# nadeemlab/DeepLIIF

Hardware: AMD Instinct MI355X
Metric: 512x512 tiles/s train-step (5G+5D) (higher is better)
Workload: dtype bf16; 1 GPU; DeepLIIF train step, 5x Resnet-9block G + 5x NLayerD(n=4), GAN+SmoothL1+Adam (BASELINE configs[2] per GPU); tile=512x512x3, batch_per_gpu=8, global_batch=8, norm=instance, precision_policy=bf16, parallelism=dp1, rccl_ranks=1, backend=nccl, streams=3

## Files before the change

deepliif_amd/csrc/wgrad.hip:

```cpp
#include "common.h"
#include <stdlib.h>

typedef __attribute__((ext_vector_type(4))) short s16x4_t;

struct WgradArgs {
    const void *P;
    const void *Q;
    float *slab;
    int kstride;
    int N, Hp, Wp, CAp, p_pstride;
    int Hq, Wq, CBp, log2CB, q_pstride;
    int KH, KW, step, pad, pad_w, pad_mode;
    int J;
    int Ptot;
    int splitk, pchunk;
    int tiles_a, tiles_j;
    int dn, dh, dw;
    int p_act, q_act;
    int xcd_group;
    int p_split, q_split;
    int tr_asm;
};

constexpr int WGRAD_MULTI_MAX = DL_WGRAD_MULTI_MAX;
// ... 601 lines not shown
    DL_CHECK_LAUNCH("dl_conv_wgrad(8-phase)");
    return 0;
}

template <int BA, int WA, int WJ, bool TRASM>
static int launch_wgrad_glds_v(WgradArgs a, const WgradLayers &lay, int n, hipStream_t stream) {
    constexpr size_t smem = (size_t)2 * 64 * (BA + 256) * sizeof(bf16_t);
    a.tiles_a = a.CAp / BA;
    a.tiles_j = (a.J + 255) / 256;
    a.pchunk = ((a.Ptot + a.splitk - 1) / a.splitk + 63) / 64 * 64;
    const int hw = a.Hp * a.Wp;
    a.dn = 64 / hw; a.dh = (64 % hw) / a.Wp; a.dw = (64 % hw) % a.Wp;
    auto kern = wgrad_glds_kernel<BA, WA, WJ, TRASM>;
    static bool attr_set = false;
    if (!attr_set) {
        hipError_t e = hipFuncSetAttribute(reinterpret_cast<const void *>(kern), hipFuncAttributeMaxDynamicSharedMemorySize, (int)smem);
        if (e != hipSuccess) DL_FAIL("dl_conv_wgrad: hipFuncSetAttribute: %s", hipGetErrorString(e));
        attr_set = true;
    }
    hipLaunchKernelGGL(kern, dim3(a.tiles_a * a.tiles_j, a.splitk, n), dim3(512), smem, stream, a, lay);
    DL_CHECK_LAUNCH("dl_conv_wgrad(glds)");
    return 0;
}

template <int BA, int WA, int WJ>
static int launch_wgrad_glds(const WgradArgs &a, const WgradLayers &lay, int n, hipStream_t stream) {
    return a.tr_asm ? launch_wgrad_glds_v<BA, WA, WJ, true>(a, lay, n, stream) : launch_wgrad_glds_v<BA, WA, WJ, false>(a, lay, n, stream);
}

__device__ __forceinline__ void wgrad_reduce_body(const float *slab, int splitk, int kstride_, int CBp, int J, int CA, int CB, int KK, float *grad,
                                                  int accumulate, int stack_kw, int bid, int nb) {
    const int J4 = J / 4;
    const size_t total = (size_t)CA * J4;
    const size_t kstride = (size_t)kstride_;
    for (size_t i = bid * (size_t)blockDim.x + threadIdx.x; i < total; i += (size_t)nb * blockDim.x) {
        const int ca = (int)(i / J4), j = (int)(i % J4) * 4;
        const float *src = slab + (size_t)ca * J + j;
        f32x4_t s = {0.f, 0.f, 0.f, 0.f};
        int k = 0;
        for (; k + 8 <= splitk; k += 8) {
            f32x4_t v[8];
#pragma unroll
            for (int u = 0; u < 8; ++u) v[u] = __builtin_nontemporal_load(reinterpret_cast<const f32x4_t *>(src + (size_t)(k + u) * kstride));
#pragma unroll
            for (int u = 0; u < 8; ++u) s += v[u];
        }
        for (; k < splitk; ++k) s += __builtin_nontemporal_load(reinterpret_cast<const f32x4_t *>(src + (size_t)k * kstride));
        const int t = j / CBp, b0 = j % CBp;
        if (t >= KK) continue;
#pragma unroll
        for (int e = 0; e < 4; ++e) {
            const int b = b0 + e;
            if (b >= CB) continue;
            float *g = stack_kw ? grad + (((size_t)(ca / stack_kw) * CB + b) * KK + t) * stack_kw + (ca % stack_kw)
                                : grad + ((size_t)ca * CB + b) * KK + t;
            *g = accumulate ? *g + s[e] : s[e];
        }
    }
}

constexpr int RED_BCHUNK = 64, RED_KK_MAX = 64, RED_MAX_BLOCKS = 8192;

__device__ __forceinline__ bool wgrad_reduce_tiled(int KK, int stack_kw) { return stack_kw == 0 && KK <= RED_KK_MAX; }

__device__ __forceinline__ void wgrad_reduce_tiles(const float *slab, int splitk, int kstride_, int CBp, int J, int CA, int CB, int KK, float *grad,
                                                   int accumulate, int bid, int nb, float *lds) {
    const int nbc = (CBp + RED_BCHUNK - 1) / RED_BCHUNK, KP = KK + 1;
    const size_t kstride = (size_t)kstride_;
    for (int item = bid; item < CA * nbc; item += nb) {
        const int ca = item / nbc, b0 = (item - ca * nbc) * RED_BCHUNK;
        const int width = min(RED_BCHUNK, CBp - b0), q = width / 4;
        const int nreal = min(width, CB - b0);
        if (nreal > 0) {
            const float *base = slab + (size_t)ca * J + b0;
            for (int i = threadIdx.x; i < KK * q; i += 256) {
                const int t = i / q, c = (i - t * q) * 4;
                const float *src = base + (size_t)t * CBp + c;
                f32x4_t s = {0.f, 0.f, 0.f, 0.f};
                int k = 0;
                for (; k + 8 <= splitk; k += 8) {
                    f32x4_t v[8];
#pragma unroll
                    for (int u = 0; u < 8; ++u) v[u] = __builtin_nontemporal_load(reinterpret_cast<const f32x4_t *>(src + (size_t)(k + u) * kstride));
#pragma unroll
                    for (int u = 0; u < 8; ++u) s += v[u];
                }
                for (; k < splitk; ++k) s += __builtin_nontemporal_load(reinterpret_cast<const f32x4_t *>(src + (size_t)k * kstride));
#pragma unroll
                for (int e = 0; e < 4; ++e) lds[(c + e) * KP + t] = s[e];
            }
        }
        __syncthreads();
        if (nreal > 0) {
            float *g = grad + ((size_t)ca * CB + b0) * KK;
            for (int o = threadIdx.x; o < nreal * KK; o += 256) {
                const float v = lds[o + o / KK];
                g[o] = accumulate ? g[o] + v : v;
            }
        }
        __syncthreads();
    }
}

__global__ void __launch_bounds__(256) wgrad_reduce_kernel(const float *slab, int splitk, int kstride, int CBp, int J, int CA, int CB,
                                                           int KK, float *grad, int accumulate, int stack_kw) {
    __shared__ float lds[RED_BCHUNK * (RED_KK_MAX + 1)];
    if (wgrad_reduce_tiled(KK, stack_kw)) wgrad_reduce_tiles(slab, splitk, kstride, CBp, J, CA, CB, KK, grad, accumulate, blockIdx.x, gridDim.x, lds);
    else wgrad_reduce_body(slab, splitk, kstride, CBp, J, CA, CB, KK, grad, accumulate, stack_kw, blockIdx.x, gridDim.x);
}

__global__ void __launch_bounds__(256) wgrad_reduce_batch_kernel(const dl_wgrad_reduce_entry *tab, int n) {
    __shared__ float lds[RED_BCHUNK * (RED_KK_MAX + 1)];
    int lo = 0, hi = n - 1;
    const int b = blockIdx.x;
    while (lo < hi) {
        const int mid = (lo + hi + 1) >> 1;
        if (tab[mid].block0 <= b) lo = mid; else hi = mid - 1;
    }
    const dl_wgrad_reduce_entry e = tab[lo];
    if (wgrad_reduce_tiled(e.KK, e.stack_kw))
        wgrad_reduce_tiles(e.slab, e.splitk, e.kstride, e.CBp, e.J, e.CA, e.CB, e.KK, e.grad, e.accumulate, b - e.block0, e.nblocks, lds);
    else wgrad_reduce_body(e.slab, e.splitk, e.kstride, e.CBp, e.J, e.CA, e.CB, e.KK, e.grad, e.accumulate, e.stack_kw, b - e.block0, e.nblocks);
}

template <typename T, int PREC, int BA, int WA, int WJ>
static int launch_wgrad(WgradArgs a, hipStream_t stream) {
    constexpr int NPL = (PREC == 3) ? 2 : 1;
    constexpr size_t smem = (size_t)2 * NPL * 32 * ((BA + 16) + (128 + 16)) * sizeof(bf16_t);
    a.tiles_a = (a.CAp + BA - 1) / BA;
    a.tiles_j = (a.J + 127) / 128;
    auto kern = wgrad_kernel<T, PREC, BA, WA, WJ>;
    static bool attr_set = false;
    if (!attr_set) {
        hipError_t e = hipFuncSetAttribute(reinterpret_cast<const void *>(kern), hipFuncAttributeMaxDynamicSharedMemorySize, (int)smem);
        if (e != hipSuccess) DL_FAIL("dl_conv_wgrad: hipFuncSetAttribute: %s", hipGetErrorString(e));
        attr_set = true;
    }
    hipLaunchKernelGGL(kern, dim3(a.tiles_a * a.tiles_j, a.splitk), dim3(256), smem, stream, a);
    DL_CHECK_LAUNCH("dl_conv_wgrad");
    return 0;
}

template <typename T, int PREC>
static int dispatch_wgrad(const WgradArgs &a, hipStream_t stream) {
    if (a.CAp <= 16) return launch_wgrad<T, PREC, 16, 1, 4>(a, stream);
    if (a.CAp <= 32) return launch_wgrad<T, PREC, 32, 1, 4>(a, stream);
    if (a.CAp <= 64) return launch_wgrad<T, PREC, 64, 2, 2>(a, stream);
    return launch_wgrad<T, PREC, 128, 2, 2>(a, stream);
}

#include "wgrad_c4.h"
#include "wgrad_x3.h"
#include "wgrad_w4.h"

static int wgrad_slab_pad() {
    static const int pad = [] { const char *e = DL_DEV_ENV("DL_WGRAD_SLAB_PAD"); const int v = e ? atoi(e) : 0; return v < 0 ? 0 : (v + 3) / 4 * 4; }();
    return pad;
}

extern "C" size_t dl_wgrad_slab_floats(const dl_wgrad_desc *d) {
    if (!d || d->splitk < 1) return 0;
    return (size_t)d->splitk * ((size_t)d->CAp * d->KH * d->KW * d->CBp + wgrad_slab_pad());
}

enum WgradKernel { WK_GENERIC = 0, WK_GLDS256, WK_GLDS128, WK_X3_256, WK_X3_128, WK_8PH, WK_4PH_X3, WK_4PH_X3_NOPRIO, WK_W4 };

static int wgrad_kernel_of(const dl_wgrad_desc *d, int *err) {
    *err = 0;
    const int J = d->KH * d->KW * d->CBp;
    const long Ptot = (long)d->N * d->Hp * d->Wp;
    static const bool no_glds = DL_DEV_ENV("DL_NO_GLDS") != nullptr;
    const bool fast = d->dtype == DL_BF16 && d->prec == DL_PREC_BF16 && d->p_act == DL_ACT_NONE && d->q_act == DL_ACT_NONE &&
                      d->pad_mode == DL_PAD_ZERO && J >= 256 && Ptot >= 64L * d->splitk && !no_glds;
    static const char *w8 = DL_DEV_ENV("DL_WGRAD_8PH");
    const bool no_x3 = dl_switch(DL_SW_NO_X3_GLDS) != nullptr;
    const bool act_ok3 = (d->p_act == DL_ACT_NONE || d->p_act == DL_ACT_RELU || d->p_act == DL_ACT_LRELU) &&
                         (d->q_act == DL_ACT_NONE || d->q_act == DL_ACT_RELU || d->q_act == DL_ACT_LRELU);
    const bool fast3 = d->dtype == DL_F32 && d->prec == DL_PREC_BF16X3 && act_ok3 && d->pad_mode == DL_PAD_ZERO && J >= 256 &&
                       Ptot >= 32L * d->splitk && (d->p_pstride % 4) == 0 && (d->q_pstride % 4) == 0 && !no_x3;
    static const char *w3 = DL_DEV_ENV("DL_WGRAD_X3");
    if ((d->p_split || d->q_split) && !(fast3 && (d->CAp % 128) == 0 && (!d->p_split || d->p_act == DL_ACT_NONE) && (!d->q_split || d->q_act == DL_ACT_NONE))) {
        *err = 1;
        return WK_GENERIC;
    }
    if (w4w_eligible(d)) return WK_W4;
    if (fast3 && (d->CAp % 256) == 0 && w3 && (w3[0] == '2' || w3[0] == '3') && !d->p_split && !d->q_split) return w3[0] == '3' ? WK_4PH_X3_NOPRIO : WK_4PH_X3;
    if (fast3 && (d->CAp % 256) == 0) return WK_X3_256;
    if (fast3 && (d->CAp % 128) == 0) return WK_X3_128;
    if (fast && (d->CAp % 256) == 0 && w8 && w8[0] == '1') return WK_8PH;
    if (fast && (d->CAp % 256) == 0) return WK_GLDS256;
    if (fast && (d->CAp % 128) == 0) return WK_GLDS128;
    return WK_GENERIC;
}

static int wgrad_slabs(const dl_wgrad_desc *d, const WgradLayers &lay, int n, hipStream_t stream, int *J_out) {
    if (!d) DL_FAIL("dl_conv_wgrad: null descriptor");
    if (d->N <= 0 || d->Hp <= 0 || d->Wp <= 0 || d->Hq <= 0 || d->Wq <= 0)
        DL_FAIL("dl_conv_wgrad: empty problem (N=%d, P %dx%d, Q %dx%d): nothing to launch", d->N, d->Hp, d->Wp, d->Hq, d->Wq);
    if (n < 1 || n > WGRAD_MULTI_MAX) DL_FAIL("dl_conv_wgrad: %d layers in one launch (1 .. %d)", n, WGRAD_MULTI_MAX);
    for (int l = 0; l < n; ++l)
        if (!lay.P[l] || !lay.Q[l] || !lay.slab[l]) DL_FAIL("dl_conv_wgrad: null argument");
    const int l2 = ilog2_exact(d->CBp);
    if (l2 < 3) DL_FAIL("dl_conv_wgrad: CBp=%d must be a power of two >= 8", d->CBp);
    if (d->CAp % 8) DL_FAIL("dl_conv_wgrad: CAp=%d must be a multiple of 8", d->CAp);
    if (d->p_pstride % 8 || d->q_pstride % 8) DL_FAIL("dl_conv_wgrad: pixel strides must be multiples of 8");
    if (d->splitk < 1) DL_FAIL("dl_conv_wgrad: splitk=%d", d->splitk);
    if (d->stack_kw && d->KW != 1) DL_FAIL("dl_conv_wgrad: stack_kw needs KW == 1");
    if (d->prec == DL_PREC_BF16X3 && d->dtype != DL_F32) DL_FAIL("dl_conv_wgrad: BF16X3 needs fp32 activations");
    if (d->pad_mode < DL_PAD_ZERO || d->pad_mode > DL_PAD_REPLICATE) DL_FAIL("dl_conv_wgrad: pad_mode=%d (0 zero | 1 reflect | 2 replicate)", d->pad_mode);
    if (d->pad_mode == DL_PAD_REPLICATE && d->step != 1) DL_FAIL("dl_conv_wgrad: replicate padding only for step == 1 layers (step=%d)", d->step);

    WgradArgs a;
    memset(&a, 0, sizeof(a));
    a.P = lay.P[0]; a.Q = lay.Q[0]; a.slab = lay.slab[0];
    a.N = d->N; a.Hp = d->Hp; a.Wp = d->Wp; a.CAp = d->CAp; a.p_pstride = d->p_pstride;
    a.Hq = d->Hq; a.Wq = d->Wq; a.CBp = d->CBp; a.log2CB = l2; a.q_pstride = d->q_pstride;
    a.KH = d->KH; a.KW = d->KW; a.step = d->step; a.pad = d->pad; a.pad_w = d->pad_w < 0 ? d->pad : d->pad_w; a.pad_mode = d->pad_mode;
    a.J = d->KH * d->KW * d->CBp;
    a.kstride = d->CAp * a.J + wgrad_slab_pad();
    a.Ptot = d->N * d->Hp * d->Wp;
    a.splitk = d->splitk;
    a.pchunk = ((a.Ptot + d->splitk - 1) / d->splitk + 31) / 32 * 32;
    const int hw = d->Hp * d->Wp;
    a.dn = 32 / hw; a.dh = (32 % hw) / d->Wp; a.dw = (32 % hw) % d->Wp;
    a.p_act = d->p_act; a.q_act = d->q_act;
    a.p_split = d->p_split; a.q_split = d->q_split;
    static const char *tr_env = DL_DEV_ENV("DL_WGRAD_TR_ASM");
    a.tr_asm = (tr_env && tr_env[0] == '0') ? 0 : 1;
    static const char *xg_env = DL_DEV_ENV("DL_WGRAD_XCDGROUP");
    a.xcd_group = (xg_env && xg_env[0] == '0') ? 0 : 1;

    int err = 0;
    const int k = wgrad_kernel_of(d, &err);
    if (err)
        DL_FAIL("dl_conv_wgrad: split-copy operands need the strict direct-to-LDS kernel (fp32 + BF16X3, zero padding, CAp %% 128 == 0, J >= 256) and no staged activation on them");
    if (n > 1 && !(k == WK_W4 || k == WK_GLDS256 || k == WK_GLDS128 || k == WK_X3_256 || k == WK_X3_128))
        DL_FAIL("dl_conv_wgrad_multi: this descriptor takes a kernel without a batched form (ask dl_wgrad_plan first)");
    int rc;
    switch (k) {
        case WK_W4: rc = launch_wgrad_w4(d, lay, n, a.kstride, stream); break;
        case WK_4PH_X3: rc = launch_wgrad_4ph_x3<0>(a, stream); break;
        case WK_4PH_X3_NOPRIO: rc = launch_wgrad_4ph_x3<1>(a, stream); break;
        case WK_X3_256: rc = launch_wgrad_glds_x3<256>(a, lay, n, stream); break;
        case WK_X3_128: rc = launch_wgrad_glds_x3<128>(a, lay, n, stream); break;
        case WK_8PH: rc = launch_wgrad_8ph(a, stream); break;
        case WK_GLDS256: rc = launch_wgrad_glds<256, 2, 4>(a, lay, n, stream); break;
        case WK_GLDS128: rc = launch_wgrad_glds<128, 2, 4>(a, lay, n, stream); break;
        default:
            if (d->dtype == DL_BF16 && d->prec == DL_PREC_BF16) rc = dispatch_wgrad<bf16_t, 1>(a, stream);
            else if (d->dtype == DL_F32 && d->prec == DL_PREC_BF16X3) rc = dispatch_wgrad<float, 3>(a, stream);
            else if (d->dtype == DL_F32 && d->prec == DL_PREC_BF16) rc = dispatch_wgrad<float, 1>(a, stream);
            else DL_FAIL("dl_conv_wgrad: unsupported dtype/precision combination");
    }
    *J_out = a.J;
    return rc;
}

static int wgrad_slabs(const dl_wgrad_desc *d, const void *P, const void *Q, float *slab, hipStream_t stream, int *J_out) {
    if (!P || !Q || !slab) DL_FAIL("dl_conv_wgrad: null argument");
    WgradLayers lay;
    lay.P[0] = P; lay.Q[0] = Q; lay.slab[0] = slab;
    return wgrad_slabs(d, lay, 1, stream, J_out);
}

extern "C" int dl_wgrad_plan(const dl_wgrad_desc *d, int32_t *tiles, int32_t *ksteps, const char **name) {
    if (!d) DL_FAIL("dl_wgrad_plan: null descriptor");
    if (wgrad_c4_form(d) || wgrad_c4_x3_form(d)) {
        if (tiles) *tiles = 0;
        if (ksteps) *ksteps = 0;
        if (name) *name = "wgrad_c4";
        return 0;
    }
    int err = 0;
    const int k = wgrad_kernel_of(d, &err);
    const int J = d->KH * d->KW * d->CBp;
    const long Ptot = (long)d->N * d->Hp * d->Wp;
    int t = 0, ks = 0, multi = 0;
    const char *nm = "wgrad_kernel";
    switch (k) {
        case WK_W4: t = (d->CAp / 128) * (d->CBp / 128) * 3; ks = d->N * d->Hp; multi = 1; nm = "wgrad_w4_kernel"; break;
        case WK_X3_256: case WK_4PH_X3: case WK_4PH_X3_NOPRIO: t = (d->CAp / 256) * ((J + 255) / 256); ks = (int)((Ptot + 31) / 32); multi = k == WK_X3_256; nm = "wgrad_glds_x3_kernel<256>"; break;
        case WK_X3_128: t = (d->CAp / 128) * ((J + 255) / 256); ks = (int)((Ptot + 31) / 32); multi = 1; nm = "wgrad_glds_x3_kernel<128>"; break;
        case WK_GLDS256: case WK_8PH: t = (d->CAp / 256) * ((J + 255) / 256); ks = (int)((Ptot + 63) / 64); multi = k == WK_GLDS256; nm = "wgrad_glds_kernel<256>"; break;
        case WK_GLDS128: t = (d->CAp / 128) * ((J + 255) / 256); ks = (int)((Ptot + 63) / 64); multi = 1; nm = "wgrad_glds_kernel<128>"; break;
        default: {
            const int ba = d->CAp <= 16 ? 16 : (d->CAp <= 32 ? 32 : (d->CAp <= 64 ? 64 : 128));
            t = ((d->CAp + ba - 1) / ba) * ((J + 127) / 128); ks = (int)((Ptot + 31) / 32);
        }
    }
    if (tiles) *tiles = t;
    if (ksteps) *ksteps = ks;
    if (name) *name = nm;
    if (err)
        DL_FAIL("dl_wgrad_plan: split-copy operands (p_split / q_split) need the strict direct-to-LDS kernels: fp32 + BF16X3, zero padding, KH*KW*CBp >= 256, "
                "CAp %% 128 == 0, pixel strides %% 4 == 0, no staged activation on a split operand (CAp=%d, J=%d, p_split=%d, q_split=%d)", d->CAp, J, d->p_split, d->q_split);
    return multi;
}

static int reduce_blocks(const dl_wgrad_desc *d, int J) {
    if (d->stack_kw == 0 && d->KH * d->KW <= RED_KK_MAX)
        return (int)min((size_t)RED_MAX_BLOCKS, (size_t)d->CA * ((d->CBp + RED_BCHUNK - 1) / RED_BCHUNK));
    const size_t total = (size_t)d->CA * (J / 4);
    return (int)min((size_t)4096, (total + 255) / 256);
}

extern "C" int dl_conv_wgrad(const dl_wgrad_desc *d, const void *P, const void *Q, float *grad, float *slab, void *stream_) {
    hipStream_t stream = (hipStream_t)stream_;
    if (!d) DL_FAIL("dl_conv_wgrad: null descriptor");
    if (!grad) DL_FAIL("dl_conv_wgrad: null argument");
    if (d->N > 0 && d->Hp > 0 && d->Wp > 0 && P && Q && slab) {
        if (const int form = wgrad_c4_form(d)) return launch_wgrad_c4(d, form, P, Q, grad, slab, stream);
        if (const int form = wgrad_c4_x3_form(d)) return launch_wgrad_c4_x3(d, form, P, Q, grad, slab, stream);
    }
    int J = 0;
    if (const int rc = wgrad_slabs(d, P, Q, slab, stream, &J)) return rc;
    hipLaunchKernelGGL(wgrad_reduce_kernel, dim3(reduce_blocks(d, J)), dim3(256), 0, stream, slab, d->splitk, d->CAp * J + wgrad_slab_pad(), d->CBp, J, d->CA, d->CB,
                       d->KH * d->KW, grad, d->accumulate, d->stack_kw);
    DL_CHECK_LAUNCH("dl_conv_wgrad(reduce)");
    return 0;
}

extern "C" int dl_conv_wgrad_deferrable(const dl_wgrad_desc *d) {
    return d && !wgrad_c4_form(d) && !wgrad_c4_x3_form(d);
}

extern "C" int dl_conv_wgrad_slabs(const dl_wgrad_desc *d, const void *P, const void *Q, float *grad, float *slab, dl_wgrad_reduce_entry *entry_host,
                                   void *stream_) {
    hipStream_t stream = (hipStream_t)stream_;
    if (!d || !entry_host || !grad) DL_FAIL("dl_conv_wgrad_slabs: null argument");
    if (!dl_conv_wgrad_deferrable(d)) DL_FAIL("dl_conv_wgrad_slabs: the persistent narrow-channel kernels reduce in place; call dl_conv_wgrad");
    int J = 0;
    if (const int rc = wgrad_slabs(d, P, Q, slab, stream, &J)) return rc;
    dl_wgrad_reduce_entry e;
    memset(&e, 0, sizeof(e));
    e.slab = slab; e.grad = grad;
    e.splitk = d->splitk; e.CAp = d->CAp; e.CBp = d->CBp; e.J = J; e.CA = d->CA; e.CB = d->CB; e.KK = d->KH * d->KW;
    e.accumulate = d->accumulate; e.stack_kw = d->stack_kw;
    e.block0 = 0; e.nblocks = reduce_blocks(d, J); e.kstride = d->CAp * J + wgrad_slab_pad();
    *entry_host = e;
    return 0;
}

extern "C" int dl_conv_wgrad_multi(const dl_wgrad_desc *d, int n, const void *const *P, const void *const *Q, float *const *grad, float *slab,
                                   dl_wgrad_reduce_entry *entries_host, void *stream_) {
    hipStream_t stream = (hipStream_t)stream_;
    if (!d || !P || !Q || !grad || !slab || !entries_host) DL_FAIL("dl_conv_wgrad_multi: null argument");
    if (n < 1 || n > WGRAD_MULTI_MAX) DL_FAIL("dl_conv_wgrad_multi: n=%d (1 .. %d)", n, WGRAD_MULTI_MAX);
    if (!dl_conv_wgrad_deferrable(d)) DL_FAIL("dl_conv_wgrad_multi: the persistent narrow-channel kernels reduce in place; call dl_conv_wgrad");
    const size_t per_layer = dl_wgrad_slab_floats(d);
    WgradLayers lay;
    for (int l = 0; l < n; ++l) {
        if (!grad[l]) DL_FAIL("dl_conv_wgrad_multi: null gradient");
        lay.P[l] = P[l]; lay.Q[l] = Q[l]; lay.slab[l] = slab + (size_t)l * per_layer;
    }
    int J = 0;
    if (const int rc = wgrad_slabs(d, lay, n, stream, &J)) return rc;
    for (int l = 0; l < n; ++l) {
        dl_wgrad_reduce_entry e;
        memset(&e, 0, sizeof(e));
        e.slab = lay.slab[l]; e.grad = grad[l];
        e.splitk = d->splitk; e.CAp = d->CAp; e.CBp = d->CBp; e.J = J; e.CA = d->CA; e.CB = d->CB; e.KK = d->KH * d->KW;
        e.accumulate = d->accumulate; e.stack_kw = d->stack_kw;
        e.block0 = 0; e.nblocks = reduce_blocks(d, J); e.kstride = d->CAp * J + wgrad_slab_pad();
        entries_host[l] = e;
    }
    return 0;
}

extern "C" int dl_wgrad_reduce_batch(const dl_wgrad_reduce_entry *table_dev, int count, int total_blocks, void *stream_) {
    hipStream_t stream = (hipStream_t)stream_;
    if (!table_dev || count <= 0 || total_blocks <= 0) DL_FAIL("dl_wgrad_reduce_batch: empty table");
    hipLaunchKernelGGL(wgrad_reduce_batch_kernel, dim3(total_blocks), dim3(256), 0, stream, table_dev, count);
    DL_CHECK_LAUNCH("dl_wgrad_reduce_batch");
    return 0;
}
```

deepliif_amd/ops.py:

```python
from __future__ import annotations

import ctypes as C
import os
import contextlib
import threading
from typing import Optional

import torch

from . import _lib as L
from .geometry import (GatherPlan, NUM_CUS, WGRAD_C4_PARTS, choose_splitk, choose_wgrad_batch_splitk, choose_wgrad_splitk, fill_conv_desc, fill_pack_desc,
                       wgrad_batch_shape, wgrad_c4_ok, wgrad_fast_path)


def dl_dtype(t: torch.Tensor) -> int:
    if t.dtype == torch.float32:
        return L.DL_F32
    if t.dtype == torch.bfloat16 or t.dtype == torch.float16:
        return L.DL_BF16
    raise TypeError(f'engine tensors are fp32 or bf16 / fp16, got {t.dtype}')


def pstride(t: torch.Tensor) -> int:
    assert t.dim() == 4 and t.stride(3) == 1, 'NHWC view with unit channel stride expected'
# ... 233 lines not shown
        tabs = []
        for kind in range(3):
            n = int(lib.dl_spectral_blocks(C.c_void_p(base), len(jobs), kind, None))
            if n < 0:
                self.check(n, 'dl_spectral_blocks')
            tab = (C.c_int32 * (2 * max(n, 1)))()
            self.check(min(int(lib.dl_spectral_blocks(C.c_void_p(base), len(jobs), kind, C.c_void_p(C.addressof(tab)))), 0), 'dl_spectral_blocks')
            tabs.append((torch.frombuffer(tab, dtype=torch.int32).clone()[:2 * n], n))
        t = SpectralTable()
        t.count, t.scratch_floats, t.device = len(jobs), off, dev
        t.jobs_dev = torch.frombuffer(host, dtype=torch.uint8).clone().to(dev)
        t.tiles_host = tabs[0][0].view(-1, 2)
        t.tiles, t.rows, t.cols = [(tab.to(dev), n) for tab, n in tabs]
        t.subsets = {}
        return t

    def spectral_forward(self, table: 'SpectralTable', iterate: bool):
        _LAUNCH.dev = table.device
        ws = WS.get('spectral', table.scratch_floats, table.device)
        self.check(self.lib.dl_spectral_forward(_ptr(table.jobs_dev), table.count, _ptr(table.tiles[0]), table.tiles[1], _ptr(table.rows[0]), table.rows[1],
                                                _ptr(table.cols[0]), table.cols[1], _ptr(ws), 1 if iterate else 0, _stream()), 'dl_spectral_forward')

    def spectral_backward(self, table: 'SpectralTable', accumulate: bool, only=None):
        tiles = table.tiles
        if only is not None and len(only) != table.count:
            tiles = table.subsets.get(only)
            if tiles is None:
                keep = torch.isin(table.tiles_host[:, 0], torch.tensor(list(only), dtype=torch.int32))
                sub = table.tiles_host[keep].contiguous()
                tiles = table.subsets[only] = (sub.view(-1).to(table.device), int(sub.shape[0]))
        if tiles[1] == 0:
            return
        _LAUNCH.dev = table.device
        ws = WS.get('spectral', table.scratch_floats, table.device)
        self.check(self.lib.dl_spectral_backward(_ptr(table.jobs_dev), table.count, _ptr(tiles[0]), tiles[1], _ptr(ws), 1 if accumulate else 0, _stream()),
                   'dl_spectral_backward')

    def conv_forward(self, packed: PackedWeights, x: torch.Tensor, out: torch.Tensor, hq: int, wq: int, bias: Optional[torch.Tensor],
                     act: int, in_act: int, prec: int, splitk: Optional[int] = None, raw_out: bool = False, want_stats: bool = False,
                     bn=None, in_split: bool = False):
        _need_cuda(x, out, bias)
        if raw_out:
            plan = packed.plan
            n, hi, wi, cp = x.shape
            _, ho, wo, cop = out.shape
            assert out.dtype == torch.float32 and out.is_contiguous()
            d = fill_conv_desc(plan, n, hi, wi, pstride(x), ho, wo, cop, cop, hq, wq, dl_dtype(x), prec, L.ACT_NONE, in_act, 0, 1, 1)
            self.check(self.lib.dl_conv_forward(C.byref(d), _ptr(x), _ptr(packed.hi), _ptr(packed.lo), None, None, _ptr(out), None, _stream()),
                    'dl_conv_forward(raw)')
            return 0
        plan = packed.plan
        n, hi, wi, cp = x.shape
        assert cp == plan.cc_pad, (cp, plan.cc_pad)
        _, ho, wo, cop = out.shape
        auto_split = splitk is None
        if auto_split:
            splitk = choose_splitk(plan, n, hq, wq, cop)
        d = fill_conv_desc(plan, n, hi, wi, pstride(x), ho, wo, cop, pstride(out), hq, wq, dl_dtype(x), prec, act, in_act,
                           0 if bias is None else bias.numel(), splitk)
        d.in_split = 1 if in_split else 0
        assert dl_dtype(out) == d.in_dtype
        if auto_split and splitk > 1 and plan.cc_real <= 4:
            d.splitk = 1
            if self.lib.dl_conv_kernel_name(C.byref(d)).decode().startswith('conv_c4_patch'):
                splitk = 1
            else:
                d.splitk = splitk
        if auto_split and splitk > 1 and plan.pad_mode == L.PAD_REPLICATE:
            d.splitk = 1
            if self.lib.dl_conv_kernel_name(C.byref(d)) == b'conv_gemm_w4_kernel':
                splitk = 1
            else:
                d.splitk = splitk
        self._last_conv_desc = d
        slab = WS.get('conv_slab', splitk * n * ho * wo * cop, x.device) if splitk > 1 else None
        nch, part = 0, None
        if want_stats:
            nch = int(self.lib.dl_conv_stats_chunks(C.byref(d)))
            if nch > 0:
                nd = self._norm_desc(out, cop, L.NORM_BATCH, L.ACT_NONE, -1.0, 8, 8)
                nd.ext_nchunks = nch
                part = WS.get('norm_ws', self.lib.dl_norm_ws_floats(C.byref(nd)), x.device)
                WS.bump_norm_token()
        if bn is not None and bias is None and splitk == 1 and not want_stats and _BNSTATS:
            by, bstats, bact = bn
            nch = int(self.lib.dl_conv_bnstats_chunks(C.byref(d)))
            if nch > 0 and by.dtype == out.dtype == torch.bfloat16 and by.shape == out.shape:
                _need_cuda(by, bstats)
                nd = self._norm_desc(out, cop, L.NORM_BATCH, L.ACT_NONE, -1.0, 8, 8)
                nd.ext_nchunks = nch
                part = WS.get('norm_ws', self.lib.dl_norm_ws_floats(C.byref(nd)), x.device)
                WS.bump_norm_token()
                b = L.ConvBnStats(by.data_ptr(), pstride(by), bact, bstats[0].data_ptr(), bstats[1].data_ptr(), bstats[2].data_ptr(),
                                  bstats[3].data_ptr())
                self.check(self.lib.dl_conv_forward_bnstats(C.byref(d), _ptr(x), _ptr(packed.hi), _ptr(packed.lo), _ptr(out), _ptr(part),
                                                         C.byref(b), _stream()), 'dl_conv_forward_bnstats')
                return nch
            nch = 0
        self.check(self.lib.dl_conv_forward(C.byref(d), _ptr(x), _ptr(packed.hi), _ptr(packed.lo), _ptr(bias), _ptr(out), _ptr(slab),
                                         _ptr(part), _stream()), 'dl_conv_forward')
        return nch

    def conv_forward_add(self, packed: PackedWeights, x: torch.Tensor, addend: torch.Tensor, out: torch.Tensor, hq: int, wq: int, prec: int) -> bool:
        if not _CONV_ADD or x.dtype != torch.bfloat16 or addend.dtype != torch.bfloat16 or addend.shape != out.shape:
            return False
        _need_cuda(x, addend, out)
        plan = packed.plan
        n, hi, wi, cp = x.shape
        _, ho, wo, cop = out.shape
        d = fill_conv_desc(plan, n, hi, wi, pstride(x), ho, wo, cop, pstride(out), hq, wq, dl_dtype(x), prec, L.ACT_NONE, L.ACT_NONE, 0, 1)
        if not self.lib.dl_conv_add_supported(C.byref(d)):
            return False
        self._last_conv_desc = d
        self.check(self.lib.dl_conv_forward_add(C.byref(d), _ptr(x), _ptr(packed.hi), _ptr(packed.lo), _ptr(addend), pstride(addend), _ptr(out), _stream()),
                'dl_conv_forward_add')
        return True

    def conv_wgrad(self, P: torch.Tensor, Q: torch.Tensor, grad: torch.Tensor, k: int, step: int, pad: int, pad_mode: int,
                   p_act: int, q_act: int, prec: int, accumulate: bool, splitk: Optional[int] = None, stack_kw: int = 0, p_split: bool = False,
                   q_split: bool = False):
        _need_cuda(P, Q, grad)
        assert grad.dtype == torch.float32 and grad.is_contiguous()
        d = L.WgradDesc()
        d.N, d.Hp, d.Wp, d.CAp = P.shape
        d.p_pstride = pstride(P)
        _, d.Hq, d.Wq, d.CBp = Q.shape
        d.q_pstride = pstride(Q)
        d.KH = d.KW = k
        d.step, d.pad, d.pad_mode = step, pad, pad_mode
        d.CA, d.CB = grad.shape[0], grad.shape[1]
        d.pad_w, d.stack_kw = -1, 0
        if stack_kw:
            d.KW, d.pad_w, d.stack_kw, d.CA = 1, 0, stack_kw, grad.shape[0] * stack_kw
        d.dtype, d.prec = dl_dtype(P), prec
        d.accumulate = 1 if accumulate else 0
        d.p_act, d.q_act = p_act, q_act
        d.p_split, d.q_split = (1 if p_split else 0), (1 if q_split else 0)
        j = d.KH * d.KW * d.CBp
        strict = d.dtype == L.DL_F32 and prec == L.PREC_BF16X3 and not _NO_X3_GLDS
        fast = wgrad_fast_path(d.CAp, j, d.dtype == L.DL_BF16 and prec == L.PREC_BF16, p_act == L.ACT_NONE and q_act == L.ACT_NONE,
                               pad_mode == L.PAD_ZERO, strict, p_act in _X3_ACTS and q_act in _X3_ACTS)
        d.splitk = 1
        tiles, ksteps, kname = L.i32(), L.i32(), C.c_char_p()
        multi = int(self.lib.dl_wgrad_plan(C.byref(d), C.byref(tiles), C.byref(ksteps), C.byref(kname)))
        if multi < 0:
            self.check(multi, 'dl_wgrad_plan')
        w4 = kname.value == b'wgrad_w4_kernel'
        deferring = _WGRAD_DEFER and WS._thread_state().get('defer_depth', 0) > 0
        if deferring and _WGRAD_BATCH and splitk is None and multi == 1 and w4 and wgrad_batch_shape(d.KH, d.KW, d.step, d.Wp, d.Hp, d.Hq, d.CAp, d.CBp):
            self._wgrad_queued(WS._state(), d, P, Q, grad, tiles.value, ksteps.value)
            return
        if splitk is not None:
            d.splitk = splitk
        elif w4:
            d.splitk = max(1, min(NUM_CUS // tiles.value, ksteps.value))
        else:
            d.splitk = choose_wgrad_splitk(d.CAp, j, d.N * d.Hp * d.Wp, fast)
        if splitk is None and not _NO_WGRAD_C4 and self.wgrad_c4_applies(P, Q, grad, k, step, pad, pad_mode, p_act, q_act, prec, stack_kw):
            d.splitk = WGRAD_C4_PARTS
        nslab = int(self.lib.dl_wgrad_slab_floats(C.byref(d)))
        if deferring and self.lib.dl_conv_wgrad_deferrable(C.byref(d)):
            self._wgrad_deferred(WS._state(), d, P, Q, grad, nslab)
            return
        slab = WS.get('wgrad_slab', nslab, P.device)
        self.check(self.lib.dl_conv_wgrad(C.byref(d), _ptr(P), _ptr(Q), _ptr(grad), _ptr(slab), _stream()), 'dl_conv_wgrad')

    def wgrad_defer_begin(self):
        st = WS._thread_state()
        st['defer_depth'] = st.get('defer_depth', 0) + 1

    def wgrad_defer_end(self):
        st = WS._thread_state()
        try:
            if st.get('defer_depth', 0) == 1:
                self.wgrad_flush_all()
        finally:
            st['defer_depth'] = max(0, st.get('defer_depth', 0) - 1)

    def wgrad_abandon(self):
        st = WS._thread_state()
        for sub in [st] + WS.stream_states():
            sub['defer_pending'], sub['defer_queue'], sub['defer_blocks'], sub['defer_off'] = [], [], 0, 0
            sub['defer_grads'] = set()
        st['defer_depth'] = 0

    def wgrad_flush_all(self):
        self.wgrad_flush()
        for sub in WS.stream_states():
            if sub.get('defer_pending') or sub.get('defer_queue'):
                with torch.cuda.stream(sub['stream_obj']):
                    self.wgrad_flush()

    def _arena_region(self, st, need: int, device):
        arena = st.get('defer_arena')
        if arena is not None and st.get('defer_off', 0) + need > arena.numel():
            self._reduce_pending(st)
        if arena is None or arena.numel() < need or arena.device != device:
            self._reduce_pending(st)
            if arena is not None:
                Workspace.realloc_generation += 1
            arena = torch.empty(max(need, _WGRAD_ARENA_MB * (1 << 18)), dtype=torch.float32, device=device)
            st['defer_arena'], st['defer_off'] = arena, 0
        off = st.get('defer_off', 0)
        st['defer_off'] = off + need
        return arena[off:off + need]

    def _wgrad_queued(self, st, d, P, Q, grad, tiles, ksteps):
        gp = grad.data_ptr()
        if gp in st.setdefault('defer_grads', set()):
            self.wgrad_flush()
        st['defer_grads'].add(gp)
        d.splitk = choose_wgrad_batch_splitk(tiles, ksteps)
        queue = st.setdefault('defer_queue', [])
        queue.append((bytes(d), d, P, Q, grad))
        if len(queue) >= L.WGRAD_MULTI_MAX:
            self._launch_queued(st)

    def _launch_queued(self, st):
        queue = st.get('defer_queue')
        if not queue:
            return
        st['defer_queue'] = []
        groups = {}
        for item in queue:
            groups.setdefault(item[0], []).append(item)
        for items in groups.values():
            d = items[0][1]
            per_layer = int(self.lib.dl_wgrad_slab_floats(C.byref(d)))
            for i0 in range(0, len(items), L.WGRAD_MULTI_MAX):
                chunk = items[i0:i0 + L.WGRAD_MULTI_MAX]
                n = len(chunk)
                slab = self._arena_region(st, (n * per_layer + 63) // 64 * 64, chunk[0][2].device)
                arr = C.c_void_p * n
                Ps, Qs, Gs = arr(*[it[2].data_ptr() for it in chunk]), arr(*[it[3].data_ptr() for it in chunk]), arr(*[it[4].data_ptr() for it in chunk])
                ents = (L.WgradReduceEntry * n)()
                _LAUNCH.dev = chunk[0][2].device
                self.check(self.lib.dl_conv_wgrad_multi(C.byref(d), n, Ps, Qs, Gs, _ptr(slab), ents, _stream()), 'dl_conv_wgrad_multi')
                pend = st.setdefault('defer_pending', [])
                for l in range(n):
                    e = L.WgradReduceEntry.from_buffer_copy(ents[l])
                    e.block0 = st.get('defer_blocks', 0)
                    st['defer_blocks'] = e.block0 + e.nblocks
                    pend.append(e)

    def _wgrad_deferred(self, st, d, P, Q, grad, nslab):
        gp = grad.data_ptr()
        need = (nslab + 63) // 64 * 64
        if gp in st.setdefault('defer_grads', set()):
            self.wgrad_flush()
        slab = self._arena_region(st, need, P.device)
        e = L.WgradReduceEntry()
        self.check(self.lib.dl_conv_wgrad_slabs(C.byref(d), _ptr(P), _ptr(Q), _ptr(grad), _ptr(slab), C.byref(e), _stream()), 'dl_conv_wgrad_slabs')
        e.block0 = st.get('defer_blocks', 0)
        st['defer_blocks'] = e.block0 + e.nblocks
        st['defer_grads'].add(gp)
        st.setdefault('defer_pending', []).append(e)

    def wgrad_flush(self):
        st = WS._state()
        self._launch_queued(st)
        self._reduce_pending(st)
        st['defer_grads'] = set()

    def _reduce_pending(self, st):
        pend = st.get('defer_pending')
        if not pend:
            st['defer_off'] = 0
            return
        arena = st['defer_arena']
        tab = (L.WgradReduceEntry * len(pend))(*pend)
        key = bytes(tab)
        cache = st.setdefault('defer_tables', {})
        dev_tab = cache.get(key)
        if dev_tab is None:
            if len(cache) >= 512:
                cache.clear()
            dev_tab = torch.frombuffer(bytearray(key), dtype=torch.uint8).to(arena.device)
            cache[key] = dev_tab
        total = st['defer_blocks']
        st['defer_pending'], st['defer_blocks'], st['defer_off'] = [], 0, 0
        _LAUNCH.dev = arena.device
        self.check(self.lib.dl_wgrad_reduce_batch(_ptr(dev_tab), len(pend), total, _stream()), 'dl_wgrad_reduce_batch')

    supports_split = os.environ.get('DL_NO_SPLIT_COPY') is None

    def conv_takes_split(self, x, prec, in_act, pad_mode) -> bool:
        return (self.supports_split and not _NO_X3_GLDS and x.dtype == torch.float32 and prec == L.PREC_BF16X3 and in_act == L.ACT_NONE)

    def wgrad_takes_split(self, P, Q, grad, k, pad_mode, prec, stack_kw=0) -> bool:
        if not self.supports_split or _NO_X3_GLDS or stack_kw or P.dtype != torch.float32 or prec != L.PREC_BF16X3 or pad_mode != L.PAD_ZERO:
            return False
        cap, j, ptot = P.shape[3], k * k * Q.shape[3], P.shape[0] * P.shape[1] * P.shape[2]
        return cap % 128 == 0 and j >= 256 and ptot >= 32 * choose_wgrad_splitk(cap, j, ptot, True)

    def wgrad_c4_applies(self, P, Q, grad, k, step, pad, pad_mode, p_act, q_act, prec, stack_kw=0) -> bool:
        return not _NO_WGRAD_C4 and wgrad_c4_ok(P.shape[3], grad.shape[0], Q.shape[3], grad.shape[1], k, step, pad, pad_mode, P.shape[1], P.shape[2], Q.shape[1], Q.shape[2],
                           (P.dtype == torch.bfloat16 and prec == L.PREC_BF16) or (P.dtype == torch.float32 and prec == L.PREC_BF16X3 and not _NO_C4_X3),
                           p_act == L.ACT_NONE and q_act == L.ACT_NONE, bool(stack_kw))

    def _norm_desc(self, y, C_real, scope, act, momentum, z_ps, r_ps):
        d = L.NormDesc()
        d.N, d.H, d.W, d.Cp = y.shape
        d.C = C_real
        d.y_pstride, d.z_pstride, d.r_pstride = pstride(y), z_ps, r_ps
        d.dtype, d.scope, d.act = dl_dtype(y), scope, act
        d.eps, d.momentum = 1e-5, momentum
        return d
# ... 318 lines not shown
```

Measured before the change: 117.6 tiles/s.

## Add dedicated stride-2 3x3 weight-gradient kernel with direct-to-LDS pipelining

Adds a specialised wgrad kernel for bf16 3x3 stride-2 pad-1 convolutions (the downsampling layers of the generators and discriminators). Each block owns one kernel row and computes all three kernel-column taps from a single LDS staging of P and Q rows. It uses a 4-deep buffer_load_lds ring, transposed LDS reads and MFMA. Split-k is sized from the CU count, as for the w4 kernel. This replaces the generic or GLDS path for these layers, aiming to cut redundant operand loads. It adds a large, complex kernel that uses a lot of LDS and has strict eligibility rules.

```diff
diff --git a/deepliif_amd/csrc/wgrad.hip b/deepliif_amd/csrc/wgrad.hip
--- a/deepliif_amd/csrc/wgrad.hip
+++ b/deepliif_amd/csrc/wgrad.hip
@@ -777,6 +777,7 @@
 #include "wgrad_c4.h"
 #include "wgrad_x3.h"
 #include "wgrad_w4.h"
+#include "wgrad_s2.h"
 
 static int wgrad_slab_pad() {
     static const int pad = [] { const char *e = DL_DEV_ENV("DL_WGRAD_SLAB_PAD"); const int v = e ? atoi(e) : 0; return v < 0 ? 0 : (v + 3) / 4 * 4; }();
@@ -788,7 +789,7 @@
     return (size_t)d->splitk * ((size_t)d->CAp * d->KH * d->KW * d->CBp + wgrad_slab_pad());
 }
 
-enum WgradKernel { WK_GENERIC = 0, WK_GLDS256, WK_GLDS128, WK_X3_256, WK_X3_128, WK_8PH, WK_4PH_X3, WK_4PH_X3_NOPRIO, WK_W4 };
+enum WgradKernel { WK_GENERIC = 0, WK_GLDS256, WK_GLDS128, WK_X3_256, WK_X3_128, WK_8PH, WK_4PH_X3, WK_4PH_X3_NOPRIO, WK_W4, WK_S2 };
 
 static int wgrad_kernel_of(const dl_wgrad_desc *d, int *err) {
     *err = 0;
@@ -809,6 +810,7 @@
         return WK_GENERIC;
     }
     if (w4w_eligible(d)) return WK_W4;
+    if (s2w_eligible(d)) return WK_S2;
     if (fast3 && (d->CAp % 256) == 0 && w3 && (w3[0] == '2' || w3[0] == '3') && !d->p_split && !d->q_split) return w3[0] == '3' ? WK_4PH_X3_NOPRIO : WK_4PH_X3;
     if (fast3 && (d->CAp % 256) == 0) return WK_X3_256;
     if (fast3 && (d->CAp % 128) == 0) return WK_X3_128;
@@ -864,6 +866,7 @@
     int rc;
     switch (k) {
         case WK_W4: rc = launch_wgrad_w4(d, lay, n, a.kstride, stream); break;
+        case WK_S2: rc = launch_wgrad_s2(d, lay, a.kstride, stream); break;
         case WK_4PH_X3: rc = launch_wgrad_4ph_x3<0>(a, stream); break;
         case WK_4PH_X3_NOPRIO: rc = launch_wgrad_4ph_x3<1>(a, stream); break;
         case WK_X3_256: rc = launch_wgrad_glds_x3<256>(a, lay, n, stream); break;
@@ -904,6 +907,7 @@
     const char *nm = "wgrad_kernel";
     switch (k) {
         case WK_W4: t = (d->CAp / 128) * (d->CBp / 128) * 3; ks = d->N * d->Hp; multi = 1; nm = "wgrad_w4_kernel"; break;
+        case WK_S2: t = (d->CAp / 128) * (d->CBp / 64) * 3; ks = d->N * d->Hp * (d->Wp / S2W_PX); nm = "wgrad_s2_kernel"; break;
         case WK_X3_256: case WK_4PH_X3: case WK_4PH_X3_NOPRIO: t = (d->CAp / 256) * ((J + 255) / 256); ks = (int)((Ptot + 31) / 32); multi = k == WK_X3_256; nm = "wgrad_glds_x3_kernel<256>"; break;
         case WK_X3_128: t = (d->CAp / 128) * ((J + 255) / 256); ks = (int)((Ptot + 31) / 32); multi = 1; nm = "wgrad_glds_x3_kernel<128>"; break;
         case WK_GLDS256: case WK_8PH: t = (d->CAp / 256) * ((J + 255) / 256); ks = (int)((Ptot + 63) / 64); multi = k == WK_GLDS256; nm = "wgrad_glds_kernel<256>"; break;
diff --git a/deepliif_amd/csrc/wgrad_s2.h b/deepliif_amd/csrc/wgrad_s2.h
--- /dev/null
+++ b/deepliif_amd/csrc/wgrad_s2.h
@@ -0,0 +1,216 @@
+#pragma once
+
+struct WgradS2Args {
+    int NH, Hp, Hq;
+    int npc;
+    int CBp, J, kstride;
+    int p_pstride, q_pstride;
+    int p_row, q_row;
+    int splitk, rps;
+    int tiles_a, tiles_b;
+};
+
+constexpr int S2W_PX = 64;
+constexpr int S2W_P = S2W_PX * 256;
+constexpr int S2W_QPIECES = 17;
+constexpr int S2W_Q = S2W_QPIECES * 1024;
+constexpr int S2W_BUF = S2W_P + S2W_Q;
+constexpr int S2W_NB = 4;
+constexpr size_t S2W_LDS = (size_t)S2W_NB * S2W_BUF;
+static_assert(S2W_LDS <= 160 * 1024, "LDS of a CU");
+
+template <int KS>
+__global__ void __launch_bounds__(256) wgrad_s2_kernel(const WgradS2Args a, const WgradLayers lay) {
+    static_assert(KS == 3, "3x3, padding 1");
+    constexpr int NF = 2 + KS;
+    extern __shared__ __attribute__((aligned(16))) char smem_raw[];
+    w4w_lds_t *lds = (w4w_lds_t *)smem_raw;
+
+    const int tid = threadIdx.x, lane = tid & 63;
+    const int wave = __builtin_amdgcn_readfirstlane(tid >> 6);
+    const int ntile = a.tiles_a * a.tiles_b * KS;
+    const int logical = xcd_remap(blockIdx.x, gridDim.x);
+    const int tile = logical % ntile, ks = logical / ntile;
+    const int kh = tile % KS, tb = (tile / KS) % a.tiles_b, ta = tile / (KS * a.tiles_b);
+
+    const char *Pg = reinterpret_cast<const char *>(lay.P[0]) + ta * 256;
+    const int pps = a.p_pstride * 2, qps = a.q_pstride * 2;
+    const char *Qg = reinterpret_cast<const char *>(lay.Q[0]) + tb * 128 - 2 * qps;
+    float *slab = lay.slab[0] + (size_t)ks * a.kstride;
+
+    const int r_begin = min(a.NH, ks * a.rps), r_end = min(a.NH, r_begin + a.rps);
+    const int h_lo = kh == 0 ? 1 : 0, h_hi = min(a.Hp - 1, (a.Hq - kh) >> 1);
+    auto valid_from = [&](int r) __attribute__((always_inline)) {
+        while (r < r_end) {
+            const int h = r % a.Hp;
+            if (h >= h_lo && h <= h_hi) break;
+            ++r;
+        }
+        return r;
+    };
+
+    const int lq = lane >> 4, lc = lane & 15;
+    const int ch = lc ^ (lq << 2);
+    const int OOB = (int)0x80000000u;
+    const int vp = lq * pps + (ch << 4);
+    const int vq = (2 * lq + (ch >> 3)) * qps + ((ch & 7) << 4);
+    const int vq_first = lq == 0 ? OOB : vq;
+    const int vq_last = lq == 0 ? vq : OOB;
+    const __amdgpu_buffer_rsrc_t rsrc_p = __builtin_amdgcn_make_buffer_rsrc(const_cast<char *>(Pg), 0, 0x7fffffff, 0x00020000);
+    const __amdgpu_buffer_rsrc_t rsrc_q = __builtin_amdgcn_make_buffer_rsrc(const_cast<char *>(Qg), 0, 0x7fffffff, 0x00020000);
+    auto issue = [&](int r, int cw, int nb) __attribute__((always_inline)) {
+        const int n_img = r / a.Hp, h = r - n_img * a.Hp;
+        const int w0 = cw * S2W_PX;
+        const int sp = r * a.p_row + (w0 + wave * 16) * pps;
+        const int sq_row = (n_img * a.Hq + 2 * h + kh - 1) * a.q_row + 2 * w0 * qps;
+        const int sq = sq_row + wave * 32 * qps;
+        const int base = nb * S2W_BUF;
+        const int vq0 = (wave == 0 && cw == 0) ? vq_first : vq;
+#pragma unroll
+        for (int j = 0; j < 4; ++j)
+            __builtin_amdgcn_raw_ptr_buffer_load_lds(rsrc_p, (__attribute__((address_space(3))) void *)(lds + base + (wave * 4 + j) * 1024), 16, vp, sp + j * 4 * pps, 0, 0);
+#pragma unroll
+        for (int j = 0; j < 4; ++j)
+            __builtin_amdgcn_raw_ptr_buffer_load_lds(rsrc_q, (__attribute__((address_space(3))) void *)(lds + base + S2W_P + (wave * 4 + j) * 1024), 16, j == 0 ? vq0 : vq,
+                                                     sq + j * 8 * qps, 0, 0);
+        if (wave == 0)
+            __builtin_amdgcn_raw_ptr_buffer_load_lds(rsrc_q, (__attribute__((address_space(3))) void *)(lds + base + S2W_P + 16 * 1024), 16,
+                                                     vq_last, sq_row + 128 * qps, 0, 0);
+    };
+    int ir = valid_from(r_begin), iw = 0, issued = 0;
+    auto issue_next = [&]() __attribute__((always_inline)) {
+        if (ir < r_end) {
+            issue(ir, iw, issued & (S2W_NB - 1));
+            ++issued;
+            if (++iw == a.npc) { iw = 0; ir = valid_from(ir + 1); }
+        }
+    };
+
+    const int m = lane & 15, g = lane >> 4;
+    const int mr = m >> 2;
+    const int lane_b = (g & 1) * 32 + (m & 3) * 8;
+    const int wq = wave & 1, pb0 = 2 * (wave >> 1);
+    int a_addr[2], x_addr[KS];
+#pragma unroll
+    for (int i = 0; i < 2; ++i) a_addr[i] = (8 * (g >> 1) + mr) * 256 + (((pb0 + i) ^ mr) << 6) + lane_b;
+#pragma unroll
+    for (int k = 0; k < KS; ++k) {
+        const int rk = (k + 1) >> 1, gk = (k & 1) ? wq : 2 + wq;
+        x_addr[k] = S2W_P + (8 * (g >> 1) + mr + rk) * 256 + ((gk ^ ((mr + rk) & 3)) << 6) + lane_b;
+    }
+
+    w4w_f32x16_t acc[2][KS];
+#pragma unroll
+    for (int i = 0; i < 2; ++i)
+#pragma unroll
+        for (int k = 0; k < KS; ++k)
+#pragma unroll
+            for (int r = 0; r < 16; ++r) acc[i][k][r] = 0.f;
+
+    bf16x8_t FA[NF], FB[NF];
+#pragma unroll
+    for (int f = 0; f < NF; ++f)
+#pragma unroll
+        for (int e = 0; e < 8; ++e) FB[f][e] = 0;
+    auto read_frags = [&](bf16x8_t (&F)[NF], int bb, auto OFS) __attribute__((always_inline)) {
+        constexpr int ofs = decltype(OFS)::value;
+#pragma unroll
+        for (int f = 0; f < NF; ++f) {
+            const int addr = (f < 2 ? a_addr[f] : x_addr[f - 2]) + bb;
+            s16x4_t lo, hi;
+            asm volatile("ds_read_b64_tr_b16 %0, %1 offset:%2" : "=v"(lo) : "v"(addr), "n"(ofs));
+            asm volatile("ds_read_b64_tr_b16 %0, %1 offset:%2" : "=v"(hi) : "v"(addr), "n"(ofs + 1024));
+            F[f][0] = lo[0]; F[f][1] = lo[1]; F[f][2] = lo[2]; F[f][3] = lo[3];
+            F[f][4] = hi[0]; F[f][5] = hi[1]; F[f][6] = hi[2]; F[f][7] = hi[3];
+        }
+    };
+    auto frag_wait = [&](bf16x8_t (&F)[NF]) __attribute__((always_inline)) {
+        static_assert(NF == 5, "the operand list below");
+        asm volatile("s_waitcnt lgkmcnt(0)" : "+v"(F[0]), "+v"(F[1]), "+v"(F[2]), "+v"(F[3]), "+v"(F[4]));
+    };
+    auto mma = [&](const bf16x8_t (&F)[NF]) __attribute__((always_inline)) {
+#pragma unroll
+        for (int i = 0; i < 2; ++i)
+#pragma unroll
+            for (int k = 0; k < KS; ++k) acc[i][k] = dl_mfma32(F[i], F[2 + k], acc[i][k]);
+    };
+    auto substep = [&](bf16x8_t (&Fc)[NF], bf16x8_t (&Fn)[NF], int bb, auto OFS) __attribute__((always_inline)) {
+        __builtin_amdgcn_sched_barrier(0);
+        frag_wait(Fc);
+        if constexpr (decltype(OFS)::value >= 0) read_frags(Fn, bb, OFS);
+        __builtin_amdgcn_sched_barrier(0);
+        mma(Fc);
+        __builtin_amdgcn_sched_barrier(0);
+    };
+
+    issue_next(); issue_next(); issue_next();
+    for (int t = 0; t < issued; ++t) {
+        __builtin_amdgcn_sched_barrier(0);
+        if (issued - t > 2) {
+            if (wave == 0) asm volatile("s_waitcnt vmcnt(18)" ::: "memory");
+            else asm volatile("s_waitcnt vmcnt(16)" ::: "memory");
+        } else {
+            asm volatile("s_waitcnt vmcnt(0)" ::: "memory");
+        }
+        frag_wait(FB);
+        asm volatile("s_barrier" ::: "memory");
+        issue_next();
+        const int bb = (t & (S2W_NB - 1)) * S2W_BUF;
+        read_frags(FA, bb, W4WIC<0>{});
+        __builtin_amdgcn_sched_barrier(0);
+        mma(FB);
+        substep(FA, FB, bb, W4WIC<1 * 4096>{});
+        substep(FB, FA, bb, W4WIC<2 * 4096>{});
+        substep(FA, FB, bb, W4WIC<3 * 4096>{});
+    }
+    __builtin_amdgcn_sched_barrier(0);
+    frag_wait(FB);
+    mma(FB);
+    __builtin_amdgcn_sched_barrier(0);
+
+    const int lr = lane & 31, lh = lane >> 5;
+#pragma unroll
+    for (int i = 0; i < 2; ++i)
+#pragma unroll
+        for (int k = 0; k < KS; ++k) {
+            float *o = slab + (size_t)(ta * 128 + 32 * (pb0 + i) + 4 * lh) * a.J + (kh * KS + k) * a.CBp + tb * 64 + 32 * wq + lr;
+#pragma unroll
+            for (int e = 0; e < 16; ++e) o[(size_t)(8 * (e >> 2) + (e & 3)) * a.J] = acc[i][k][e];
+        }
+}
+
+static bool s2w_eligible(const dl_wgrad_desc *d) {
+    static const bool off = DL_DEV_ENV("DL_NO_WGRAD_S2") != nullptr;
+    if (off) return false;
+    if (d->dtype != DL_BF16 || d->prec != DL_PREC_BF16 || d->p_act != DL_ACT_NONE || d->q_act != DL_ACT_NONE) return false;
+    if (d->pad_mode != DL_PAD_ZERO || d->stack_kw || d->p_split || d->q_split) return false;
+    if (d->KH != 3 || d->KW != 3 || d->step != 2 || d->pad != 1 || (d->pad_w >= 0 && d->pad_w != 1)) return false;
+    if (d->N < 1 || d->Hp < 1 || d->Wp < S2W_PX || (d->Wp % S2W_PX) || d->Hq != 2 * d->Hp || d->Wq != 2 * d->Wp) return false;
+    if ((d->CAp % 128) || (d->CBp % 64) || (d->p_pstride % 8) || (d->q_pstride % 8) || d->p_pstride < d->CAp || d->q_pstride < d->CBp) return false;
+    const size_t p_rows = (size_t)d->N * d->Hp, q_rows = (size_t)d->N * d->Hq;
+    if (p_rows * d->Wp * (size_t)d->p_pstride * 2 >= ((size_t)1 << 31) || (q_rows * d->Wq + 2) * (size_t)d->q_pstride * 2 >= ((size_t)1 << 31)) return false;
+    return d->splitk >= 1 && (size_t)d->splitk <= 4 * p_rows;
+}
+
+static int launch_wgrad_s2(const dl_wgrad_desc *d, const WgradLayers &lay, int kstride, hipStream_t stream) {
+    WgradS2Args a;
+    memset(&a, 0, sizeof(a));
+    a.NH = d->N * d->Hp; a.Hp = d->Hp; a.Hq = d->Hq;
+    a.npc = d->Wp / S2W_PX;
+    a.CBp = d->CBp; a.J = 9 * d->CBp; a.kstride = kstride;
+    a.p_pstride = d->p_pstride; a.q_pstride = d->q_pstride;
+    a.p_row = d->Wp * d->p_pstride * 2; a.q_row = d->Wq * d->q_pstride * 2;
+    a.splitk = d->splitk; a.rps = (a.NH + d->splitk - 1) / d->splitk;
+    a.tiles_a = d->CAp / 128; a.tiles_b = d->CBp / 64;
+    auto kern = wgrad_s2_kernel<3>;
+    static bool attr_set = false;
+    if (!attr_set) {
+        hipError_t e = hipFuncSetAttribute(reinterpret_cast<const void *>(kern), hipFuncAttributeMaxDynamicSharedMemorySize, (int)S2W_LDS);
+        if (e != hipSuccess) DL_FAIL("dl_conv_wgrad(s2): hipFuncSetAttribute(%zu): %s", S2W_LDS, hipGetErrorString(e));
+        attr_set = true;
+    }
+    const int grid = a.tiles_a * a.tiles_b * 3 * a.splitk;
+    hipLaunchKernelGGL(kern, dim3(grid), dim3(256), S2W_LDS, stream, a, lay);
+    DL_CHECK_LAUNCH("dl_conv_wgrad(s2)");
+    return 0;
+}
diff --git a/deepliif_amd/ops.py b/deepliif_amd/ops.py
--- a/deepliif_amd/ops.py
+++ b/deepliif_amd/ops.py
@@ -409,7 +409,7 @@
             return
         if splitk is not None:
             d.splitk = splitk
-        elif w4:
+        elif w4 or kname.value == b'wgrad_s2_kernel':
             d.splitk = max(1, min(NUM_CUS // tiles.value, ksteps.value))
         else:
             d.splitk = choose_wgrad_splitk(d.CAp, j, d.N * d.Hp * d.Wp, fast)
```

Result: faster. 118.9 tiles/s, median of 6 (+1.2%).
